# DogRog/no-time-to-train

Measured on NVIDIA B200. Metric: matching_stage_images_per_s, higher is better.
Workload: dtype f32

## Files before the change

no-time-to-train_b200/csrc/common.cuh:

```cuda
#pragma once

#include <cuda_runtime.h>
#include <stdint.h>

#include <atomic>

#include "../../include/nttt_b200.h"

namespace nttt {

constexpr int kWarp = 32;
constexpr unsigned kFull = 0xffffffffu;

int cuda_fail(cudaError_t e, const char* what);
#define NTTT_CUDA(expr)                                        \
  do {                                                         \
    cudaError_t _e = (expr);                                   \
    if (_e != cudaSuccess) return ::nttt::cuda_fail(_e, #expr); \
  } while (0)
cudaError_t set_dyn_smem_impl(const void* fn, int bytes);
template <typename F>
inline cudaError_t set_dyn_smem(F* fn, int bytes) { return set_dyn_smem_impl(reinterpret_cast<const void*>(fn), bytes); }
extern thread_local bool t_low_latency;
extern thread_local bool t_chain_break;
// ... 64 lines not shown
        __syncthreads();
        other = s_x[i ^ j];
        __syncthreads();
      } else {
        other = __shfl_xor_sync(kFull, key, j);
      }
      const bool take_min = ((i & j) == 0) == ((i & k) == 0);
      key = (take_min == (other < key)) ? other : key;
    }
  }
  return key;
}

__device__ __forceinline__ float4 ld_stream(const float4* p) {
  float4 r;
  asm volatile("ld.global.nc.L1::no_allocate.v4.f32 {%0,%1,%2,%3}, [%4];"
               : "=f"(r.x), "=f"(r.y), "=f"(r.z), "=f"(r.w)
               : "l"(p));
  return r;
}

struct AxisTable {
  int in_size = 0, out_size = 0, taps = 0;
  void* slab = nullptr;
  int32_t* xmin = nullptr;
  int32_t* xsize = nullptr;
  float* w = nullptr;
  int32_t* t_lo = nullptr;
  int32_t* t_len = nullptr;
  float* t_w = nullptr;
  float* t_cum = nullptr;
  int32_t* grp_of = nullptr;
  int32_t* grp_start = nullptr;
  float4* pk = nullptr;
};
constexpr int kGrpMax = 4;
constexpr int kMaxScatter = 24;

int aa_max_taps(int in_size, int out_size);

constexpr int kMaxChunks = 64;
struct ChunkTable {
  const float* base[kMaxChunks];
};

int build_axis_table(AxisTable& t, int in_size, int out_size, cudaStream_t s);
void free_axis_table(AxisTable& t);

}

struct nttt_ctx {
  int device = 0;
  int sm_count = 0;
  static constexpr int kMaxTables = 1024;
  static constexpr int kMaxRetired = 64;
  nttt::AxisTable tables[kMaxTables];
  unsigned long long last_use[kMaxTables] = {};
  nttt::AxisTable retired[kMaxRetired];
  int n_retired = 0;
  int max_tables = kMaxTables;
  unsigned long long epoch = 0;
  int n_tables = 0;
  int upsample_stage_floats = 36 * 1024 / 4;
  bool pool_order = true;
  int32_t* scratch = nullptr;
  size_t scratch_cap = 0;
  static constexpr int kMaxStages = 16;
// ... 20 lines not shown
```

no-time-to-train_b200/csrc/fullres.cu:

```cuda
#include "common.cuh"

namespace nttt {

constexpr int kUpThreads = 128;
constexpr int kUpMaxSplit = 8;
constexpr int kUpCols = 8;
constexpr int kUpSub = 32 / kUpCols;
constexpr int kUpGroupsPerCta = 32;

struct UpTables {
  const int32_t* xmin; const int32_t* xsize; const float* wx; int tx;
  const int32_t* ymin; const int32_t* ysize; const float* wy; int ty;
  const int32_t* x_tlo; const int32_t* x_tlen;
  const int32_t* y_tlo; const int32_t* y_tlen;
  const int32_t* y_grp_of; const int32_t* y_grp_start;
  const float4* pk_x; const float4* pk_y;
};

__device__ __forceinline__ float aa_dot(const float* __restrict__ src, int stride, const float* __restrict__ w, int n) {
  float acc = __fmul_rn(__ldg(src), __ldg(w));
  for (int j = 1; j < n; ++j) acc = __fmaf_rn(__ldg(src + (size_t)j * stride), __ldg(w + j), acc);
  return acc;
}

constexpr int kScratchInts = 8;
constexpr int kBig = 1 << 30;
constexpr int kTapsReg = 4;

struct alignas(16) UpMeta {
  const float* logits;
  int src;
  int safe;
  int r0, r1;
  int w0, w1;
  int lr0, lr1;
  int g0, g1;
};

__global__ void __launch_bounds__(256)
upsample_meta_kernel(const uint32_t* __restrict__ bits_lr, const int32_t* __restrict__ box_lr,
                     const int32_t* __restrict__ flags_lr, int ih, int iw, const int32_t* __restrict__ sel,
                     const int32_t* __restrict__ n_sel, int max_sel, UpTables t, UpMeta* __restrict__ meta,
                     int32_t* __restrict__ rect, int32_t* __restrict__ scratch, const float* __restrict__ logits,
                     const float* const* __restrict__ mask_ptr) {
  const int k = blockIdx.x * blockDim.x + threadIdx.x;
  if (k >= max_sel) return;
#pragma unroll
  for (int q = 0; q < kScratchInts; ++q) scratch[(size_t)k * kScratchInts + q] = 0;
  if (k >= min(*n_sel, max_sel)) return;
// ... 32 lines not shown
}
__device__ __forceinline__ void cp_async_wait_all() { asm volatile("cp.async.wait_all;" ::: "memory"); }

__global__ void __launch_bounds__(kUpThreads, 5)
upsample_pack_kernel(const uint32_t* __restrict__ bits_lr, const UpMeta* __restrict__ meta, int ih, int iw,
                     const int32_t* __restrict__ n_sel, int max_sel, int oh, int ow, UpTables t,
                     uint32_t* __restrict__ bits_full, int32_t* __restrict__ area_full, int32_t* __restrict__ box_full,
                     int32_t* __restrict__ scratch, int stage_floats) {
  extern __shared__ __align__(16) uint32_t s_lr[];
  __shared__ int s_red[5];
  const int k = blockIdx.y;
  if (k >= min(*n_sel, max_sel)) return;
  const UpMeta mt = meta[k];
  const int n_groups = mt.g1 - mt.g0;
  const int needed = up_ctas_needed(n_groups);
  if ((int)blockIdx.x >= needed) return;
  const int lr_wpr = iw >> 5;
  const int ow_words = (ow + 31) >> 5;
  const int lane = lane_id(), warp = warp_id();
  constexpr int kWarps = kUpThreads / 32;
  const int r0 = mt.r0, r1 = mt.r1, w0 = mt.w0, w1 = mt.w1;
  const int chunk0 = mt.g0 + blockIdx.x * kUpGroupsPerCta;
  const bool one_chunk = needed * kUpGroupsPerCta >= n_groups;

  int clr0 = mt.lr0, clr1 = mt.lr1;
  if (one_chunk && chunk0 < mt.g1) {
    const int gl = min(chunk0 + kUpGroupsPerCta, mt.g1);
    const int ya = max(t.y_grp_start[chunk0], r0), yb = min(t.y_grp_start[gl], r1);
    clr0 = t.ymin[ya];
    clr1 = t.ymin[yb - 1] + t.ysize[yb - 1];
  }
  const uint32_t* lr = bits_lr + ((size_t)mt.src * ih + clr0) * lr_wpr;
  const int n_lr = (clr1 - clr0) * lr_wpr;
  const bool fast_cfg = t.pk_x != nullptr && t.pk_y != nullptr;
  const float* src = mt.logits;
  float* tile = reinterpret_cast<float*>(s_lr + (((ih * lr_wpr + 1) + 3) & ~3));
  int tc0 = 0, tstride = 0;
  bool staged = false;
  if (fast_cfg && one_chunk && chunk0 < mt.g1 && stage_floats > 0 && w1 > w0) {
    const int xa = min(w0 << 5, ow - 1), xb = min((w1 << 5) - 1, ow - 1);
    tc0 = t.xmin[xa] & ~3;
    tstride = min((t.xmin[xb] + t.xsize[xb] + 3) & ~3, iw) - tc0;
    staged = tstride > 0 && (clr1 - clr0) * tstride <= stage_floats;
  }
  if (staged) {
    const int cpr = tstride >> 2;
    const int n_chunks = (clr1 - clr0) * cpr;
    const float* g0p = src + (size_t)clr0 * iw + tc0;
    for (int i = threadIdx.x; i < n_chunks; i += kUpThreads) {
      const int row = i / cpr, c4 = (i - row * cpr) << 2;
      cp_async16(tile + row * tstride + c4, g0p + (size_t)row * iw + c4);
    }
  }
  for (int i = threadIdx.x; i < n_lr; i += kUpThreads) s_lr[i] = lr[i];
  if (threadIdx.x < 5) s_red[threadIdx.x] = 0;
  const bool safe = mt.safe != 0;
  const float* tap_base = staged ? tile - clr0 * tstride : src;
  const int tap_stride = staged ? tstride : iw;
  const int tap_c0 = staged ? tc0 : 0;
  uint32_t* dst = bits_full + (size_t)k * oh * ow_words;
  cp_async_wait_all();
  __syncthreads();

  int area = 0, minx = kBig, maxx = -1, miny = kBig, maxy = -1;
  const int q = lane / kUpCols;
  for (int wbase = w0; wbase < w1; wbase += kUpCols) {
    const int wi = wbase + (lane & (kUpCols - 1));
    const bool active = wi < w1;
    const int x0 = min(wi << 5, ow - 1);
    const int x1 = min(x0 + 31, ow - 1);
    const uint32_t valid = (x1 - x0 == 31) ? 0xffffffffu : ((1u << (x1 - x0 + 1)) - 1u);
    const int c0 = t.xmin[x0];
    const int c1 = t.xmin[x1] + t.xsize[x1];
    const int cw0 = c0 >> 5;
    const bool two_words = ((c1 - 1) >> 5) <= cw0 + 1;
    uint32_t m0, m1 = 0;
    {
      const int lo = c0 - (cw0 << 5), hi = min(c1 - (cw0 << 5), 32);
      m0 = (hi - lo == 32) ? 0xffffffffu : (((1u << (hi - lo)) - 1u) << lo);
      const int hi1 = c1 - ((cw0 + 1) << 5);
      if (hi1 > 0) m1 = hi1 >= 32 ? 0xffffffffu : ((1u << hi1) - 1u);
    }
    uint32_t colbits = 0;
    for (int cb = chunk0; cb < mt.g1; cb += needed * kUpGroupsPerCta) {
      const int cend = min(cb + kUpGroupsPerCta, mt.g1);
      for (int g0 = cb + warp; g0 < cend; g0 += kWarps * kUpSub) {
        const int g = g0 + kWarps * q;
        const bool gvalid = g < cend;
        const int ya = gvalid ? max(t.y_grp_start[g], r0) : r0, yb = gvalid ? min(t.y_grp_start[g + 1], r1) : r0;
        const int nrows = yb - ya;
        int ry0, rys;
        if (fast_cfg) {
          const int pky = __float_as_int(__ldg(t.pk_y + (uint32_t)ya).x);
          ry0 = pky & 0xffff;
          rys = pky >> 16;
        } else {
          ry0 = t.ymin[ya];
          rys = t.ysize[ya];
        }
        const int rb = ry0 * tap_stride - tap_c0;
        const int lrb = (ry0 - clr0) * lr_wpr + cw0;
        uint32_t words[kGrpMax];
#pragma unroll
        for (int j = 0; j < kGrpMax; ++j) words[j] = 0;
        bool mixed = false;
        if (active && gvalid) {
          bool all0 = true, all1 = true;
          if (two_words) {
            uint32_t any = 0, miss = 0;
            if (rys <= 3) {
#pragma unroll
              for (int r = 0; r < 3; ++r) {
                if (r < rys) {
                  const uint32_t v0 = s_lr[(uint32_t)(lrb + r * lr_wpr)] & m0;
                  const uint32_t v1 = s_lr[(uint32_t)(lrb + r * lr_wpr + 1)] & m1;
                  any |= v0 | v1;
                  miss |= (v0 ^ m0) | (v1 ^ m1);
                }
              }
            } else {
              for (int r = 0; r < rys; ++r) {
                const uint32_t v0 = s_lr[lrb + r * lr_wpr] & m0;
                const uint32_t v1 = s_lr[lrb + r * lr_wpr + 1] & m1;
                any |= v0 | v1;
                miss |= (v0 ^ m0) | (v1 ^ m1);
              }
            }
            all0 = any == 0;
            all1 = miss == 0;
          } else {
            for (int r = 0; r < rys; ++r) {
              const uint32_t* row = s_lr + (lrb - cw0) + r * lr_wpr;
              for (int cw = cw0; cw <= (c1 - 1) >> 5; ++cw) {
                const int lo = max(c0 - (cw << 5), 0), hi = min(c1 - (cw << 5), 32);
                const uint32_t m = (hi - lo == 32) ? 0xffffffffu : (((1u << (hi - lo)) - 1u) << lo);
                const uint32_t v = row[cw] & m;
                all0 = all0 && (v == 0);
                all1 = all1 && (v == m);
              }
            }
          }
          if (all1 && safe && !all0) {
#pragma unroll
            for (int j = 0; j < kGrpMax; ++j) words[j] = valid;
          } else if (!all0) {
            mixed = true;
          }
        }
        uint32_t todo = __ballot_sync(kFull, mixed);
        while (todo) {
          const int src_lane = __ffs(todo) - 1;
          todo &= todo - 1;
          const int s_ya = __shfl_sync(kFull, ya, src_lane), s_nrows = __shfl_sync(kFull, nrows, src_lane);
          const int s_rb = __shfl_sync(kFull, rb, src_lane), s_rys = __shfl_sync(kFull, rys, src_lane);
          const int x = ((wbase + (src_lane & (kUpCols - 1))) << 5) + lane;
          if (fast_cfg) {
            const float4 xt = __ldg(t.pk_x + (uint32_t)x);
            const int pk = __float_as_int(xt.x);
            const int cx = pk & 0xffff, cs = pk >> 16;
            float T[3];
#pragma unroll
            for (int r = 0; r < 3; ++r) {
              float acc = 0.0f;
              if (r < s_rys) {
                const float* pl = tap_base + (s_rb + max(cx, tap_c0) + r * tap_stride);
                acc = __fmul_rn(*pl, xt.y);
                if (cs > 1) acc = __fmaf_rn(pl[1], xt.z, acc);
                if (cs > 2) acc = __fmaf_rn(pl[2], xt.w, acc);
              }
              T[r] = acc;
            }
#pragma unroll
            for (int j = 0; j < kGrpMax; ++j) {
              const float4 wv = __ldg(t.pk_y + (uint32_t)min(s_ya + j, s_ya + s_nrows - 1));
              float acc = __fmul_rn(T[0], wv.y);
              acc = __fmaf_rn(T[1], wv.z, acc);
              acc = __fmaf_rn(T[2], wv.w, acc);
              const uint32_t res = __ballot_sync(kFull, cs > 0 && acc > 0.0f);
              if (lane == src_lane) words[j] = res;
            }
            continue;
          }
          const bool inb = x < ow;
          const int cx = inb ? t.xmin[x] : 0, cs = inb ? t.xsize[x] : 1;
          const float* wx = t.wx + (size_t)(inb ? x : 0) * t.tx;
          const float* p = src + (s_rb + cx);
          if (s_rys <= kTapsReg) {
            float T[kTapsReg];
#pragma unroll
            for (int r = 0; r < kTapsReg; ++r) T[r] = (r < s_rys && inb) ? aa_dot(p + (size_t)r * iw, 1, wx, cs) : 0.0f;
#pragma unroll
            for (int j = 0; j < kGrpMax; ++j) {
              if (j < s_nrows) {
                const float* wy = t.wy + (size_t)(s_ya + j) * t.ty;
                float acc = __fmul_rn(T[0], __ldg(wy));
#pragma unroll
                for (int r = 1; r < kTapsReg; ++r)
                  if (r < s_rys) acc = __fmaf_rn(T[r], __ldg(wy + r), acc);
                const uint32_t res = __ballot_sync(kFull, inb && acc > 0.0f);
                if (lane == src_lane) words[j] = res;
              }
            }
          } else {
#pragma unroll
            for (int j = 0; j < kGrpMax; ++j) {
              if (j < s_nrows) {
                const float* wy = t.wy + (size_t)(s_ya + j) * t.ty;
                float acc = 0.0f;
                if (inb) {
                  acc = __fmul_rn(aa_dot(p, 1, wx, cs), __ldg(wy));
// ... 204 lines not shown
      const int tc0 = __ldg(t.xmin + xa) & ~3;
      const int tstride = min((__ldg(t.xmin + xb) + __ldg(t.xsize + xb) + 3) & ~3, iw) - tc0;
      Up2Item it;
      it.k = k0 + lo;
      it.g = gA | ((gB - gA) << 16);
      it.w = wA | ((wB - wA) << 16);
      it.y = ya | ((yb - ya) << 16);
      it.lr = l0 | ((l1 - l0) << 16);
      it.tc = tc0 | (tstride << 16);
      it.staged = (l1 - l0) * tstride <= tile_cap_floats ? 1 : 0;
      it.pad = 0;
      items[base + e] = it;
    }
    base += strip_items;
    __syncthreads();
  }
  if (blockIdx.x == 0 && tid == 0) { ctr[0] = base; ctr[1] = 0; }
}

__device__ __forceinline__ void cp_async16_ca(void* smem_dst, const void* gmem_src) {
  const uint32_t d = (uint32_t)__cvta_generic_to_shared(smem_dst);
  asm volatile("cp.async.ca.shared.global [%0], [%1], 16;" ::"r"(d), "l"(gmem_src) : "memory");
}
__device__ __forceinline__ void cp_async4(void* smem_dst, const void* gmem_src) {
  const uint32_t d = (uint32_t)__cvta_generic_to_shared(smem_dst);
  asm volatile("cp.async.ca.shared.global [%0], [%1], 4;" ::"r"(d), "l"(gmem_src) : "memory");
}
__device__ __forceinline__ float lds_f32(uint32_t saddr) {
  float v;
  asm volatile("ld.shared.f32 %0, [%1];" : "=f"(v) : "r"(saddr));
  return v;
}

template <bool kStaged>
__device__ __forceinline__ float up2_row(const float* __restrict__ gsrc, uint32_t saddr, int idx, const float4& xt, int cs) {
  float a0, a1 = 0.0f, a2 = 0.0f;
  if (kStaged) {
    const uint32_t p = saddr + ((uint32_t)idx << 2);
    a0 = lds_f32(p);
    if (cs > 1) a1 = lds_f32(p + 4);
    if (cs > 2) a2 = lds_f32(p + 8);
  } else {
    const float* p = gsrc + idx;
    a0 = __ldg(p);
    if (cs > 1) a1 = __ldg(p + 1);
    if (cs > 2) a2 = __ldg(p + 2);
  }
  float acc = __fmul_rn(a0, xt.y);
  acc = __fmaf_rn(a1, xt.z, acc);
  acc = __fmaf_rn(a2, xt.w, acc);
  return acc;
}

struct alignas(16) Up2Group { int row, nrows, trow, rys; };

template <bool kStaged>
__device__ __forceinline__ void up2_evaluate(int warp, int lane, int n_list, const uint16_t* __restrict__ s_list,
                                             const Up2Group* __restrict__ s_grp, const float4* __restrict__ s_pkx,
                                             const float4* __restrict__ s_pky, uint32_t* __restrict__ s_out,
                                             const float* __restrict__ gsrc, uint32_t tile_saddr, int tap_stride,
                                             int tap_c0) {
  constexpr int kWarps = kUp2Threads / 32;
  for (int e = warp; e < n_list; e += kWarps) {
    const int ent = s_list[e];
    const int u = ent >> 5, gl = ent & 31;
    const Up2Group g = s_grp[gl];
    const float4 xt = s_pkx[(u << 5) + lane];
    const int pk = __float_as_int(xt.x);
    const int cx = pk & 0xffff, cs = pk >> 16;
    const int idx = g.trow + max(cx - tap_c0, 0);
    const float T0 = up2_row<kStaged>(gsrc, tile_saddr, idx, xt, cs);
    float T1 = 0.0f, T2 = 0.0f;
    if (g.rys > 1) T1 = up2_row<kStaged>(gsrc, tile_saddr, idx + tap_stride, xt, cs);
    if (g.rys > 2) T2 = up2_row<kStaged>(gsrc, tile_saddr, idx + 2 * tap_stride, xt, cs);
    const float4* wy = s_pky + g.row;
    uint32_t mine = 0;
#pragma unroll
    for (int j = 0; j < kGrpMax; ++j) {
      const float4 wv = wy[j];
      float acc = __fmul_rn(T0, wv.y);
      acc = __fmaf_rn(T1, wv.z, acc);
      acc = __fmaf_rn(T2, wv.w, acc);
      const uint32_t res = __ballot_sync(kFull, cs > 0 && acc > 0.0f);
      if (lane == j) mine = res;
    }
    if (lane < g.nrows) {
      const int row = g.row + lane;
      s_out[u * kUp2OutStride + row + (row >> 5)] = mine;
    }
  }
}

__global__ void __launch_bounds__(kUp2Threads, kUp2CtasPerSm)
upsample_pack2_kernel(const uint32_t* __restrict__ bits_lr, const UpMeta* __restrict__ meta, int ih, int iw, int oh,
                      int ow, UpTables t, uint32_t* __restrict__ bits_full, uint32_t* __restrict__ bits_t,
                      int32_t* __restrict__ area_full, int32_t* __restrict__ box_full, int32_t* __restrict__ scratch,
                      const Up2Item* __restrict__ items, int32_t* __restrict__ ctr, int32_t* __restrict__ zero2) {
  chain_wait();
  if (zero2 && blockIdx.x == 0 && threadIdx.x == 0) { zero2[0] = 0; zero2[1] = 0; }
  extern __shared__ __align__(16) unsigned char s_raw[];
  float4* s_pkx = reinterpret_cast<float4*>(s_raw);
  float4* s_pky = s_pkx + kUp2Cols * 32;
  Up2Group* s_grp = reinterpret_cast<Up2Group*>(s_pky + kUp2Rows + kGrpMax);
  uint32_t* s_out = reinterpret_cast<uint32_t*>(s_grp + kUp2Groups);
  int* s_gstart = reinterpret_cast<int*>(s_out + kUp2Cols * kUp2OutStride);
  uint16_t* s_list = reinterpret_cast<uint16_t*>(s_gstart + kUp2Groups + 4);
  const int lr_wpr = iw >> 5;
  uint32_t* s_lr = reinterpret_cast<uint32_t*>(s_list + kUp2Cols * kUp2Groups);
  float* tile = reinterpret_cast<float*>(s_lr + ((ih * lr_wpr + 4 + 3) & ~3));
  __shared__ int s_item;
  __shared__ int s_red[5];
  __shared__ uint32_t s_mix[kUp2Cols];
  const int tid = threadIdx.x, lane = tid & 31, warp = tid >> 5;
  constexpr int kWarps = kUp2Threads / 32;
  const int ow_words = (ow + 31) >> 5;
  const int total = ctr[0];
  const uint32_t tile_saddr = (uint32_t)__cvta_generic_to_shared(tile);
  for (;;) {
    __syncthreads();
    if (tid == 0) s_item = atomicAdd(&ctr[1], 1);
    if (tid < 5) s_red[tid] = 0;
    __syncthreads();
    const int item = s_item;
    if (item >= total) break;
    const Up2Item it = items[item];
    const int k = it.k;
    const UpMeta mt = meta[k];
    const int gA = it.g & 0xffff, ng = it.g >> 16;
    const int wA = it.w & 0xffff, nw = it.w >> 16;
    const int ya0 = it.y & 0xffff, n_rows = it.y >> 16;
    const int clr0 = it.lr & 0xffff, tr = it.lr >> 16;
    const int tc0 = it.tc & 0xffff, tstride = it.tc >> 16;
    const bool staged = it.staged != 0;
    const float* src = mt.logits;
    if (staged) {
      const int cpr = tstride >> 2;
      const float* gp = src + (size_t)(clr0 + warp) * iw + tc0 + (lane << 2);
      uint32_t sp = tile_saddr + (uint32_t)((warp * tstride + (lane << 2)) << 2);
      const uint32_t sp_step = (uint32_t)(kWarps * tstride) << 2;
      const size_t gp_step = (size_t)kWarps * iw;
      for (int row = warp; row < tr; row += kWarps, gp += gp_step, sp += sp_step)
        for (int c = lane; c < cpr; c += 32)
          asm volatile("cp.async.cg.shared.global [%0], [%1], 16;" ::"r"(sp + ((uint32_t)(c - lane) << 4)), "l"(gp + ((c - lane) << 2)) : "memory");
    }
    {
      const uint32_t* lr = bits_lr + ((size_t)mt.src * ih + clr0) * lr_wpr;
      const int n_lr = tr * lr_wpr;
      if ((lr_wpr & 3) == 0 && (reinterpret_cast<uintptr_t>(lr) & 15) == 0) {
        for (int i = tid; i < (n_lr >> 2); i += kUp2Threads) cp_async16_ca(s_lr + 4 * i, lr + 4 * i);
      } else {
        for (int i = tid; i < n_lr; i += kUp2Threads) cp_async4(s_lr + i, lr + i);
      }
      for (int i = tid; i < n_rows; i += kUp2Threads) cp_async16_ca(s_pky + i, t.pk_y + ya0 + i);
      const float4* px = t.pk_x + (wA << 5);
      for (int i = tid; i < (nw << 5); i += kUp2Threads) cp_async16_ca(s_pkx + i, px + i);
      if (tid <= ng) s_gstart[tid] = min(max(t.y_grp_start[gA + tid], mt.r0), mt.r1);
    }
    cp_async_wait_all();
    __syncthreads();
    const int tap_stride = staged ? tstride : iw;
    const int tap_c0 = staged ? tc0 : 0;
    const bool safe = mt.safe != 0;
    int my_ya = 0, my_nrows = 0, my_ry0 = 0, my_rys = 0;
    if (lane < ng) {
      my_ya = s_gstart[lane];
      my_nrows = s_gstart[lane + 1] - my_ya;
      if (my_nrows > 0) {
        const int pky = __float_as_int(s_pky[my_ya - ya0].x);
        my_ry0 = pky & 0xffff;
        my_rys = pky >> 16;
      }
      if (warp == 0) {
        Up2Group g;
        g.row = my_ya - ya0;
        g.nrows = my_nrows;
        g.trow = (staged ? my_ry0 - clr0 : my_ry0) * tap_stride;
        g.rys = my_rys;
        s_grp[lane] = g;
      }
    }
    for (int u = warp; u < nw; u += kWarps) {
      const int wi = wA + u;
      const int x0 = min(wi << 5, ow - 1);
      const int x1 = min(x0 + 31, ow - 1);
      const uint32_t valid = (x1 - x0 == 31) ? 0xffffffffu : ((1u << (x1 - x0 + 1)) - 1u);
      const int p0 = __float_as_int(s_pkx[x0 - (wA << 5)].x), p1 = __float_as_int(s_pkx[x1 - (wA << 5)].x);
      const int c0 = p0 & 0xffff;
      const int c1 = (p1 & 0xffff) + (p1 >> 16);
      const int cw0 = c0 >> 5;
      const bool two_words = ((c1 - 1) >> 5) <= cw0 + 1;
      uint32_t m0, m1 = 0;
      {
        const int lo = c0 - (cw0 << 5), hi = min(c1 - (cw0 << 5), 32);
        m0 = (hi - lo == 32) ? 0xffffffffu : (((1u << (hi - lo)) - 1u) << lo);
        const int hi1 = c1 - ((cw0 + 1) << 5);
        if (hi1 > 0) m1 = hi1 >= 32 ? 0xffffffffu : ((1u << hi1) - 1u);
      }
      int cls = 0;
      if (my_nrows > 0) {
        const int lrb = (my_ry0 - clr0) * lr_wpr + cw0;
        bool all0 = true, all1 = true;
        if (two_words) {
          uint32_t any = 0, miss = 0;
          for (int r = 0; r < my_rys; ++r) {
            const uint32_t v0 = s_lr[lrb + r * lr_wpr] & m0;
            const uint32_t v1 = s_lr[lrb + r * lr_wpr + 1] & m1;
            any |= v0 | v1;
            miss |= (v0 ^ m0) | (v1 ^ m1);
          }
          all0 = any == 0;
          all1 = miss == 0;
        } else {
          for (int r = 0; r < my_rys; ++r) {
            const uint32_t* row = s_lr + (lrb - cw0) + r * lr_wpr;
            for (int cw = cw0; cw <= (c1 - 1) >> 5; ++cw) {
              const int lo = max(c0 - (cw << 5), 0), hi = min(c1 - (cw << 5), 32);
              const uint32_t m = (hi - lo == 32) ? 0xffffffffu : (((1u << (hi - lo)) - 1u) << lo);
              const uint32_t v = row[cw] & m;
              all0 = all0 && (v == 0);
              all1 = all1 && (v == m);
            }
          }
        }
        cls = all0 ? 0 : ((all1 && safe) ? 1 : 2);
        if (cls != 2) {
          const uint32_t word = cls == 1 ? valid : 0u;
          const int row = my_ya - ya0;
          for (int j = 0; j < my_nrows; ++j) s_out[u * kUp2OutStride + (row + j) + ((row + j) >> 5)] = word;
        }
      }
      const uint32_t mixed = __ballot_sync(kFull, cls == 2);
      if (lane == 0) s_mix[u] = mixed;
    }
    __syncthreads();
    int n_list = 0;
    {
      int off = 0;
      for (int u = 0; u < nw; ++u) {
        const uint32_t mixed = s_mix[u];
        if ((u & (kWarps - 1)) == warp && ((mixed >> lane) & 1u))
          s_list[off + __popc(mixed & ((1u << lane) - 1u))] = (uint16_t)((u << 5) | lane);
        off += __popc(mixed);
      }
      n_list = off;
    }
    __syncthreads();
    if (staged)
      up2_evaluate<true>(warp, lane, n_list, s_list, s_grp, s_pkx, s_pky, s_out, src, tile_saddr, tap_stride, tap_c0);
    else
      up2_evaluate<false>(warp, lane, n_list, s_list, s_grp, s_pkx, s_pky, s_out, src, tile_saddr, tap_stride, tap_c0);
    __syncthreads();
    if (bits_t) {
      uint32_t* dt = bits_t + (size_t)k * oh * ow_words;
      for (int c = warp; c < nw; c += kWarps)
        for (int row = lane; row < n_rows; row += 32)
          dt[(uint32_t)((wA + c) * oh + ya0 + row)] = s_out[c * kUp2OutStride + row + (row >> 5)];
    }
    {
      uint32_t* dst = bits_full ? bits_full + (size_t)k * oh * ow_words : nullptr;
      const int c = tid & (kUp2Cols - 1);
      int area = 0, miny = kBig, maxy = -1;
      uint32_t colbits = 0;
      if (c < nw) {
        for (int row = tid >> 3; row < n_rows; row += kUp2Threads / kUp2Cols) {
          const uint32_t w = s_out[c * kUp2OutStride + row + (row >> 5)];
          if (dst) dst[(uint32_t)((ya0 + row) * ow_words + wA + c)] = w;
          area += __popc(w);
          colbits |= w;
          if (w) { miny = min(miny, ya0 + row); maxy = max(maxy, ya0 + row); }
        }
      }
      int minx = kBig, maxx = -1;
      if (colbits) {
        minx = ((wA + c) << 5) + __ffs(colbits) - 1;
        maxx = ((wA + c) << 5) + 31 - __clz(colbits);
      }
      area = warp_sum(area);
      minx = warp_min(minx); miny = warp_min(miny); maxx = warp_max(maxx); maxy = warp_max(maxy);
      if (lane == 0) {
        atomicAdd(&s_red[0], area);
        atomicMax(&s_red[1], maxx + 1);
        atomicMax(&s_red[2], maxy + 1);
        atomicMax(&s_red[3], kBig - minx);
        atomicMax(&s_red[4], kBig - miny);
      }
    }
    __syncthreads();
    if (tid == 0) {
      int32_t* sc = scratch + (size_t)k * kScratchInts;
      atomicAdd(&sc[0], s_red[0]);
      atomicMax(&sc[1], s_red[1]);
      atomicMax(&sc[2], s_red[2]);
      atomicMax(&sc[3], s_red[3]);
      atomicMax(&sc[4], s_red[4]);
      __threadfence();
      const int prev = atomicAdd(&sc[5], 1);
      if (prev == sc[6] - 1) {
        __threadfence();
        const int a = atomicAdd(&sc[0], 0);
        const int mx1 = atomicMax(&sc[1], 0), my1 = atomicMax(&sc[2], 0);
        const int bx = atomicMax(&sc[3], 0), by = atomicMax(&sc[4], 0);
        area_full[k] = a;
        int4 o = make_int4(0, 0, 0, 0);
        if (a > 0) o = make_int4(kBig - bx, kBig - by, mx1 - 1, my1 - 1);
        reinterpret_cast<int4*>(box_full)[k] = o;
      }
    }
  }
}

static size_t up2_fixed_smem(int ih, int iw) {
  const size_t lr_words = (((size_t)ih * (iw / 32) + 4) + 3) & ~(size_t)3;
  return sizeof(float4) * (kUp2Cols * 32 + kUp2Rows + kGrpMax + kUp2Groups) +
         4 * ((size_t)kUp2Cols * kUp2OutStride + kUp2Groups + 4 + lr_words) + 2 * (size_t)kUp2Cols * kUp2Groups;
}
static size_t up2_max_items(int max_sel, int oh, int ow) {
  return (size_t)max_sel * ((oh + kUp2Groups - 1) / kUp2Groups) * ((((ow + 31) / 32) + kUp2Cols - 1) / kUp2Cols);
}

int launch_upsample_pack(const AxisTable& tx, const AxisTable& ty, const float* logits, const uint32_t* bits_lr,
                         const int32_t* box_lr, const int32_t* flags_lr, int ih, int iw, const int32_t* sel,
                         const int32_t* n_sel, int max_sel, int oh, int ow, uint32_t* bits_full, int32_t* rect,
                         int32_t* area_full, int32_t* box_full, int32_t* scratch, const float* const* mask_ptr,
                         cudaStream_t s, int stage_floats, int sm_count, uint32_t* bits_t, bool* wrote_t, bool t_only,
                         bool low_latency, int32_t* zero2) {
  if (wrote_t) *wrote_t = false;
  if (max_sel <= 0) return NTTT_OK;
  if (iw % 32 != 0) return NTTT_EUNSUPPORTED;
  UpTables t{tx.xmin, tx.xsize, tx.w, tx.taps, ty.xmin, ty.xsize, ty.w, ty.taps, tx.t_lo, tx.t_len, ty.t_lo, ty.t_len,
             ty.grp_of, ty.grp_start, tx.pk, ty.pk};
  UpMeta* meta = reinterpret_cast<UpMeta*>(scratch + (size_t)kScratchInts * max_sel);
  if (tx.pk && ty.pk && oh < 65536 && ow < 65536 && ih * (iw / 32) <= 16384) {
    int32_t* ctr = reinterpret_cast<int32_t*>(meta + max_sel);
    Up2Item* items = reinterpret_cast<Up2Item*>(ctr + 4);
    const double sy = (double)ih / oh, sx = (double)iw / ow;
    long need = (long)((kUp2Rows * sy + 6)) * (long)(((kUp2Cols * 32) * sx + 12));
    int tile_floats = (int)(need < stage_floats ? need : stage_floats);
    if (tile_floats < 0) tile_floats = 0;
    tile_floats = (tile_floats + 3) & ~3;
    const size_t smem = up2_fixed_smem(ih, iw) + (size_t)tile_floats * 4;
    if (smem > 200 * 1024) return NTTT_EUNSUPPORTED;
    launch_chain(upsample_plan_kernel, 8, kPlanThreads, 0, s, bits_lr, box_lr, flags_lr, ih, iw, sel, n_sel, max_sel, t, meta, rect,
                                                    scratch, logits, mask_ptr, items, ctr, area_full, box_full, oh, ow,
                                                    tile_floats);
    NTTT_LAUNCH_CHECK();
    if (smem > 48 * 1024)
      NTTT_CUDA(set_dyn_smem(upsample_pack2_kernel, (int)smem));
    const int grid = (sm_count > 0 ? sm_count : 148) * (low_latency ? kUp2CtasPerSm : 1);
    launch_chain(upsample_pack2_kernel, grid, kUp2Threads, smem, s, bits_lr, meta, ih, iw, oh, ow, t,
                                                          (bits_t && t_only) ? nullptr : bits_full, bits_t, area_full,
                                                          box_full, scratch, items, ctr, zero2);
    NTTT_LAUNCH_CHECK();
    if (wrote_t) *wrote_t = bits_t != nullptr;
    return NTTT_OK;
  }
  const size_t bits_bytes = ((((size_t)ih * (iw / 32) + 1) + 3) & ~(size_t)3) * 4;
  if (bits_bytes > 160 * 1024) return NTTT_EUNSUPPORTED;
  size_t stage_bytes = (size_t)(stage_floats > 0 ? stage_floats : 0) * 4;
  if (bits_bytes + stage_bytes > 200 * 1024) stage_bytes = 0;
  const size_t smem = bits_bytes + stage_bytes;
  if (smem > 48 * 1024)
    NTTT_CUDA(set_dyn_smem(upsample_pack_kernel, (int)smem));
  upsample_meta_kernel<<<ceil_div(max_sel, 256), 256, 0, s>>>(bits_lr, box_lr, flags_lr, ih, iw, sel, n_sel, max_sel, t,
                                                              meta, rect, scratch, logits, mask_ptr);
  NTTT_LAUNCH_CHECK();
// ... 133 lines not shown
```

no-time-to-train_b200/csrc/lowres.cu:

```cuda
#include <cuda_bf16.h>
#include <stdlib.h>

#include "common.cuh"

namespace nttt {

constexpr int kPackThreads = 256;
constexpr int kPackBlock = kPackThreads + 32;
constexpr int kPackStages = 4;
constexpr int kPackStageF4 = 4 * kPackThreads;
constexpr int kPackStageBytes = kPackStageF4 * 16;

__device__ __forceinline__ uint32_t pk_smem_u32(const void* p) { return (uint32_t)__cvta_generic_to_shared(p); }
__device__ __forceinline__ void pk_mbar_init(uint64_t* bar, uint32_t count) {
  asm volatile("mbarrier.init.shared::cta.b64 [%0], %1;" ::"r"(pk_smem_u32(bar)), "r"(count));
}
__device__ __forceinline__ void pk_mbar_expect_tx(uint32_t bar_addr, uint32_t bytes) {
  asm volatile("mbarrier.arrive.expect_tx.shared::cta.b64 _, [%0], %1;" ::"r"(bar_addr), "r"(bytes) : "memory");
}
__device__ __forceinline__ void pk_mbar_arrive(uint32_t bar_addr) {
  asm volatile("mbarrier.arrive.shared::cta.b64 _, [%0];" ::"r"(bar_addr) : "memory");
}
__device__ __forceinline__ void pk_mbar_wait(uint32_t bar_addr, uint32_t parity) {
  for (uint32_t spin = 0; spin < (1u << 20); ++spin) {
    uint32_t done;
    asm volatile(
        "{\n\t.reg .pred p;\n\t"
        "mbarrier.try_wait.parity.shared::cta.b64 p, [%1], %2, %3;\n\t"
        "selp.u32 %0, 1, 0, p;\n\t}"
        : "=r"(done)
        : "r"(bar_addr), "r"(parity), "r"(4000u)
        : "memory");
    if (done) return;
  }
// ... 583 lines not shown
    }
  }
  const int len = lo < 0 ? 0 : hi - lo + 1;
  t_lo[e] = max(lo, 0);
  t_len[e] = len;
  for (int t = 0; t < kMaxScatter; ++t) {
    const int x = lo + t;
    float v = 0.0f;
    if (lo >= 0 && x <= hi && e >= xmin[x] && e < xmin[x] + xsize[x]) v = w[(size_t)x * taps + (e - xmin[x])];
    t_w[(size_t)e * kMaxScatter + t] = v;
  }
  float c = 0.0f;
  t_cum[(size_t)e * (kMaxScatter + 1)] = 0.0f;
  for (int t = 0; t < kMaxScatter; ++t) {
    c += t_w[(size_t)e * kMaxScatter + t];
    t_cum[(size_t)e * (kMaxScatter + 1) + t + 1] = c;
  }
}

__global__ void aa_group_kernel(int out_size, const int32_t* xmin, const int32_t* xsize, int32_t* grp_of,
                                int32_t* grp_start) {
  if (blockIdx.x != 0 || threadIdx.x != 0) return;
  int g = -1, run = 0;
  for (int i = 0; i < out_size; ++i) {
    const bool same = i > 0 && xmin[i] == xmin[i - 1] && xsize[i] == xsize[i - 1] && run < kGrpMax;
    if (!same) { ++g; grp_start[g] = i; run = 0; }
    grp_of[i] = g;
    ++run;
  }
  for (int k = g + 1; k <= out_size; ++k) grp_start[k] = out_size;
}

__global__ void aa_pack_kernel(int out_size, int out_pad, int taps, const int32_t* xmin, const int32_t* xsize,
                               const float* w, float4* pk) {
  const int i = blockIdx.x * blockDim.x + threadIdx.x;
  if (i >= out_pad) return;
  float4 e = make_float4(0.f, 0.f, 0.f, 0.f);
  if (i < out_size) {
    const int cs = xsize[i];
    const float* wi = w + (size_t)i * taps;
    e.x = __int_as_float(xmin[i] | (cs << 16));
    e.y = cs > 0 ? wi[0] : 0.0f;
    e.z = cs > 1 ? wi[1] : 0.0f;
    e.w = cs > 2 ? wi[2] : 0.0f;
  }
  pk[i] = e;
}

int build_axis_table(AxisTable& t, int in_size, int out_size, cudaStream_t s) {
  t.in_size = in_size;
  t.out_size = out_size;
  t.taps = aa_max_taps(in_size, out_size);
  const bool packed = t.taps <= 3 && in_size < 65536;
  const int out_pad = (out_size + 31) / 32 * 32;
  size_t off = 0;
  auto take = [&](size_t bytes) { const size_t o = off; off = align_up(off + bytes, 256); return o; };
  const size_t o_xmin = take(sizeof(int32_t) * out_size), o_xsize = take(sizeof(int32_t) * out_size);
  const size_t o_w = take(sizeof(float) * (size_t)out_size * t.taps);
  const size_t o_tlo = take(sizeof(int32_t) * in_size), o_tlen = take(sizeof(int32_t) * in_size);
  const size_t o_tw = take(sizeof(float) * (size_t)in_size * kMaxScatter);
  const size_t o_tcum = take(sizeof(float) * (size_t)in_size * (kMaxScatter + 1));
  const size_t o_gof = take(sizeof(int32_t) * out_size), o_gst = take(sizeof(int32_t) * ((size_t)out_size + 1));
  const size_t o_pk = packed ? take(sizeof(float4) * (size_t)out_pad) : 0;
  char* slab = nullptr;
  NTTT_CUDA(cudaMalloc(&slab, off));
  t.slab = slab;
  t.xmin = reinterpret_cast<int32_t*>(slab + o_xmin);
  t.xsize = reinterpret_cast<int32_t*>(slab + o_xsize);
  t.w = reinterpret_cast<float*>(slab + o_w);
  t.t_lo = reinterpret_cast<int32_t*>(slab + o_tlo);
  t.t_len = reinterpret_cast<int32_t*>(slab + o_tlen);
  t.t_w = reinterpret_cast<float*>(slab + o_tw);
  t.t_cum = reinterpret_cast<float*>(slab + o_tcum);
  t.grp_of = reinterpret_cast<int32_t*>(slab + o_gof);
  t.grp_start = reinterpret_cast<int32_t*>(slab + o_gst);
  t.pk = packed ? reinterpret_cast<float4*>(slab + o_pk) : nullptr;
  aa_table_kernel<<<ceil_div(out_size, 128), 128, 0, s>>>(in_size, out_size, t.taps, t.xmin, t.xsize, t.w);
  NTTT_LAUNCH_CHECK();
  aa_transpose_kernel<<<ceil_div(in_size, 128), 128, 0, s>>>(in_size, out_size, t.taps, t.xmin, t.xsize, t.w, t.t_lo,
                                                            t.t_len, t.t_w, t.t_cum);
  NTTT_LAUNCH_CHECK();
  aa_group_kernel<<<1, 32, 0, s>>>(out_size, t.xmin, t.xsize, t.grp_of, t.grp_start);
  NTTT_LAUNCH_CHECK();
  if (packed) {
    aa_pack_kernel<<<ceil_div(out_pad, 128), 128, 0, s>>>(out_size, out_pad, t.taps, t.xmin, t.xsize, t.w, t.pk);
    NTTT_LAUNCH_CHECK();
  }
  return NTTT_OK;
}

void free_axis_table(AxisTable& t) {
  if (t.slab) cudaFree(t.slab);
  t = AxisTable{};
}

constexpr int kProjThreads = 256;

struct ProjTables {
  const int32_t* x_lo; const int32_t* x_len; const float* x_cum;
  const int32_t* y_lo; const int32_t* y_len; const float* y_w;
};

__device__ __forceinline__ void split_bf16_pair(float x, __nv_bfloat16& hi, __nv_bfloat16& lo) {
  hi = __float2bfloat16_rn(x);
  lo = __float2bfloat16_rn(x - __bfloat162float(hi));
}

constexpr int kCum = kMaxScatter + 1;
constexpr int kProjRows = 64;

template <typename F>
__device__ __forceinline__ void warp_range(int n, F flag, int& lo, int& hi) {
  const int lane = lane_id();
  const uint32_t b0 = __ballot_sync(kFull, lane < n && flag(lane));
  const uint32_t b1 = __ballot_sync(kFull, lane + 32 < n && flag(lane + 32));
  lo = b0 ? __ffs(b0) - 1 : (b1 ? 32 + __ffs(b1) - 1 : 1);
  hi = b1 ? 63 - __clz(b1) : (b0 ? 31 - __clz(b0) : 0);
}
// ... 227 lines not shown
```

Measured before the change: 12080.

## Split packed resize tables into span and 2-tap weights; defer scratch publish

Replaces the float4 packed axis table with a separate uint32 span array and a float2 weight array. The packed path is now enabled only when every output's support spans at most two input taps, so the upsample evaluation drops the third tap and does fewer loads and FMAs. The persistent upsample loop now prefetches the next work item early and defers the global atomic publish of the previous item so it overlaps the next item's loads. The bits_t and bits_full store passes are also merged with the area and box reduction. In exchange, the fast path covers fewer scale configurations, and the host-side float check must match the device tap computation exactly.

```diff
diff --git a/no-time-to-train_b200/csrc/common.cuh b/no-time-to-train_b200/csrc/common.cuh
--- a/no-time-to-train_b200/csrc/common.cuh
+++ b/no-time-to-train_b200/csrc/common.cuh
@@ -120,7 +120,8 @@
   float* t_cum = nullptr;
   int32_t* grp_of = nullptr;
   int32_t* grp_start = nullptr;
-  float4* pk = nullptr;
+  uint32_t* pk_span = nullptr;
+  float2* pk_w = nullptr;
 };
 constexpr int kGrpMax = 4;
 constexpr int kMaxScatter = 24;
diff --git a/no-time-to-train_b200/csrc/fullres.cu b/no-time-to-train_b200/csrc/fullres.cu
--- a/no-time-to-train_b200/csrc/fullres.cu
+++ b/no-time-to-train_b200/csrc/fullres.cu
@@ -14,7 +14,7 @@
   const int32_t* x_tlo; const int32_t* x_tlen;
   const int32_t* y_tlo; const int32_t* y_tlen;
   const int32_t* y_grp_of; const int32_t* y_grp_start;
-  const float4* pk_x; const float4* pk_y;
+  const uint32_t* pkx_span; const float2* pkx_w; const uint32_t* pky_span; const float2* pky_w;
 };
 
 __device__ __forceinline__ float aa_dot(const float* __restrict__ src, int stride, const float* __restrict__ w, int n) {
@@ -113,7 +113,7 @@
   }
   const uint32_t* lr = bits_lr + ((size_t)mt.src * ih + clr0) * lr_wpr;
   const int n_lr = (clr1 - clr0) * lr_wpr;
-  const bool fast_cfg = t.pk_x != nullptr && t.pk_y != nullptr;
+  const bool fast_cfg = t.pkx_span != nullptr && t.pky_span != nullptr;
   const float* src = mt.logits;
   float* tile = reinterpret_cast<float*>(s_lr + (((ih * lr_wpr + 1) + 3) & ~3));
   int tc0 = 0, tstride = 0;
@@ -172,7 +172,7 @@
         const int nrows = yb - ya;
         int ry0, rys;
         if (fast_cfg) {
-          const int pky = __float_as_int(__ldg(t.pk_y + (uint32_t)ya).x);
+          const int pky = (int)__ldg(t.pky_span + (uint32_t)ya);
           ry0 = pky & 0xffff;
           rys = pky >> 16;
         } else {
@@ -236,27 +236,25 @@
           const int s_rb = __shfl_sync(kFull, rb, src_lane), s_rys = __shfl_sync(kFull, rys, src_lane);
           const int x = ((wbase + (src_lane & (kUpCols - 1))) << 5) + lane;
           if (fast_cfg) {
-            const float4 xt = __ldg(t.pk_x + (uint32_t)x);
-            const int pk = __float_as_int(xt.x);
+            const float2 xt = __ldg(t.pkx_w + (uint32_t)x);
+            const int pk = (int)__ldg(t.pkx_span + (uint32_t)x);
             const int cx = pk & 0xffff, cs = pk >> 16;
-            float T[3];
-#pragma unroll
-            for (int r = 0; r < 3; ++r) {
+            float T[2];
+#pragma unroll
+            for (int r = 0; r < 2; ++r) {
               float acc = 0.0f;
               if (r < s_rys) {
                 const float* pl = tap_base + (s_rb + max(cx, tap_c0) + r * tap_stride);
-                acc = __fmul_rn(*pl, xt.y);
-                if (cs > 1) acc = __fmaf_rn(pl[1], xt.z, acc);
-                if (cs > 2) acc = __fmaf_rn(pl[2], xt.w, acc);
+                acc = __fmul_rn(*pl, xt.x);
+                if (cs > 1) acc = __fmaf_rn(pl[1], xt.y, acc);
               }
               T[r] = acc;
             }
 #pragma unroll
             for (int j = 0; j < kGrpMax; ++j) {
-              const float4 wv = __ldg(t.pk_y + (uint32_t)min(s_ya + j, s_ya + s_nrows - 1));
-              float acc = __fmul_rn(T[0], wv.y);
-              acc = __fmaf_rn(T[1], wv.z, acc);
-              acc = __fmaf_rn(T[2], wv.w, acc);
+              const float2 wv = __ldg(t.pky_w + (uint32_t)min(s_ya + j, s_ya + s_nrows - 1));
+              float acc = __fmul_rn(T[0], wv.x);
+              acc = __fmaf_rn(T[1], wv.y, acc);
               const uint32_t res = __ballot_sync(kFull, cs > 0 && acc > 0.0f);
               if (lane == src_lane) words[j] = res;
             }
@@ -527,55 +525,49 @@
   return v;
 }
 
+
 template <bool kStaged>
-__device__ __forceinline__ float up2_row(const float* __restrict__ gsrc, uint32_t saddr, int idx, const float4& xt, int cs) {
-  float a0, a1 = 0.0f, a2 = 0.0f;
+__device__ __forceinline__ float up2_row(const float* __restrict__ gsrc, uint32_t saddr, int idx, const float2& wx, int cs) {
+  float a0, a1 = 0.0f;
   if (kStaged) {
     const uint32_t p = saddr + ((uint32_t)idx << 2);
     a0 = lds_f32(p);
     if (cs > 1) a1 = lds_f32(p + 4);
-    if (cs > 2) a2 = lds_f32(p + 8);
   } else {
     const float* p = gsrc + idx;
     a0 = __ldg(p);
     if (cs > 1) a1 = __ldg(p + 1);
-    if (cs > 2) a2 = __ldg(p + 2);
-  }
-  float acc = __fmul_rn(a0, xt.y);
-  acc = __fmaf_rn(a1, xt.z, acc);
-  acc = __fmaf_rn(a2, xt.w, acc);
-  return acc;
+  }
+  return __fmaf_rn(a1, wx.y, __fmul_rn(a0, wx.x));
 }
 
 struct alignas(16) Up2Group { int row, nrows, trow, rys; };
 
 template <bool kStaged>
 __device__ __forceinline__ void up2_evaluate(int warp, int lane, int n_list, const uint16_t* __restrict__ s_list,
-                                             const Up2Group* __restrict__ s_grp, const float4* __restrict__ s_pkx,
-                                             const float4* __restrict__ s_pky, uint32_t* __restrict__ s_out,
-                                             const float* __restrict__ gsrc, uint32_t tile_saddr, int tap_stride,
-                                             int tap_c0) {
+                                             const Up2Group* __restrict__ s_grp, const uint32_t* __restrict__ s_xspan,
+                                             const float2* __restrict__ s_xw, const float2* __restrict__ s_yw,
+                                             uint32_t* __restrict__ s_out, const float* __restrict__ gsrc,
+                                             uint32_t tile_saddr, int tap_stride, int tap_c0) {
   constexpr int kWarps = kUp2Threads / 32;
   for (int e = warp; e < n_list; e += kWarps) {
     const int ent = s_list[e];
     const int u = ent >> 5, gl = ent & 31;
     const Up2Group g = s_grp[gl];
-    const float4 xt = s_pkx[(u << 5) + lane];
-    const int pk = __float_as_int(xt.x);
+    const int px = (u << 5) + lane;
+    const int pk = (int)s_xspan[px];
+    const float2 wx = s_xw[px];
     const int cx = pk & 0xffff, cs = pk >> 16;
     const int idx = g.trow + max(cx - tap_c0, 0);
-    const float T0 = up2_row<kStaged>(gsrc, tile_saddr, idx, xt, cs);
-    float T1 = 0.0f, T2 = 0.0f;
-    if (g.rys > 1) T1 = up2_row<kStaged>(gsrc, tile_saddr, idx + tap_stride, xt, cs);
-    if (g.rys > 2) T2 = up2_row<kStaged>(gsrc, tile_saddr, idx + 2 * tap_stride, xt, cs);
-    const float4* wy = s_pky + g.row;
+    const float T0 = up2_row<kStaged>(gsrc, tile_saddr, idx, wx, cs);
+    const float T1r = up2_row<kStaged>(gsrc, tile_saddr, idx + (g.rys > 1 ? tap_stride : 0), wx, cs);
+    const float T1 = g.rys > 1 ? T1r : 0.0f;
+    const float2* wy = s_yw + g.row;
     uint32_t mine = 0;
 #pragma unroll
     for (int j = 0; j < kGrpMax; ++j) {
-      const float4 wv = wy[j];
-      float acc = __fmul_rn(T0, wv.y);
-      acc = __fmaf_rn(T1, wv.z, acc);
-      acc = __fmaf_rn(T2, wv.w, acc);
+      const float2 wv = wy[j];
+      const float acc = __fmaf_rn(T1, wv.y, __fmul_rn(T0, wv.x));
       const uint32_t res = __ballot_sync(kFull, cs > 0 && acc > 0.0f);
       if (lane == j) mine = res;
     }
@@ -583,6 +575,28 @@
       const int row = g.row + lane;
       s_out[u * kUp2OutStride + row + (row >> 5)] = mine;
     }
+  }
+}
+
+__device__ __forceinline__ void up2_publish(int k, const int (&red)[5], int32_t* __restrict__ scratch,
+                                            int32_t* __restrict__ area_full, int32_t* __restrict__ box_full) {
+  int32_t* sc = scratch + (size_t)k * kScratchInts;
+  atomicAdd(&sc[0], red[0]);
+  atomicMax(&sc[1], red[1]);
+  atomicMax(&sc[2], red[2]);
+  atomicMax(&sc[3], red[3]);
+  atomicMax(&sc[4], red[4]);
+  __threadfence();
+  const int prev = atomicAdd(&sc[5], 1);
+  if (prev == sc[6] - 1) {
+    __threadfence();
+    const int a = atomicAdd(&sc[0], 0);
+    const int mx1 = atomicMax(&sc[1], 0), my1 = atomicMax(&sc[2], 0);
+    const int bx = atomicMax(&sc[3], 0), by = atomicMax(&sc[4], 0);
+    area_full[k] = a;
+    int4 o = make_int4(0, 0, 0, 0);
+    if (a > 0) o = make_int4(kBig - bx, kBig - by, mx1 - 1, my1 - 1);
+    reinterpret_cast<int4*>(box_full)[k] = o;
   }
 }
 
@@ -594,9 +608,11 @@
   chain_wait();
   if (zero2 && blockIdx.x == 0 && threadIdx.x == 0) { zero2[0] = 0; zero2[1] = 0; }
   extern __shared__ __align__(16) unsigned char s_raw[];
-  float4* s_pkx = reinterpret_cast<float4*>(s_raw);
-  float4* s_pky = s_pkx + kUp2Cols * 32;
-  Up2Group* s_grp = reinterpret_cast<Up2Group*>(s_pky + kUp2Rows + kGrpMax);
+  float2* s_xw = reinterpret_cast<float2*>(s_raw);
+  float2* s_yw = s_xw + kUp2Cols * 32;
+  uint32_t* s_xspan = reinterpret_cast<uint32_t*>(s_yw + kUp2Rows + 8);
+  uint32_t* s_yspan = s_xspan + kUp2Cols * 32;
+  Up2Group* s_grp = reinterpret_cast<Up2Group*>(s_yspan + kUp2Rows + 4);
   uint32_t* s_out = reinterpret_cast<uint32_t*>(s_grp + kUp2Groups);
   int* s_gstart = reinterpret_cast<int*>(s_out + kUp2Cols * kUp2OutStride);
   uint16_t* s_list = reinterpret_cast<uint16_t*>(s_gstart + kUp2Groups + 4);
@@ -611,13 +627,14 @@
   const int ow_words = (ow + 31) >> 5;
   const int total = ctr[0];
   const uint32_t tile_saddr = (uint32_t)__cvta_generic_to_shared(tile);
+  int next = 0, pend_k = -1, pend[5];
+  if (tid == 0) s_item = atomicAdd(&ctr[1], 1);
   for (;;) {
-    __syncthreads();
-    if (tid == 0) s_item = atomicAdd(&ctr[1], 1);
-    if (tid < 5) s_red[tid] = 0;
     __syncthreads();
     const int item = s_item;
     if (item >= total) break;
+    if (tid == 0) next = atomicAdd(&ctr[1], 1);
+    if (tid < 5) s_red[tid] = 0;
     const Up2Item it = items[item];
     const int k = it.k;
     const UpMeta mt = meta[k];
@@ -646,11 +663,14 @@
       } else {
         for (int i = tid; i < n_lr; i += kUp2Threads) cp_async4(s_lr + i, lr + i);
       }
-      for (int i = tid; i < n_rows; i += kUp2Threads) cp_async16_ca(s_pky + i, t.pk_y + ya0 + i);
-      const float4* px = t.pk_x + (wA << 5);
-      for (int i = tid; i < (nw << 5); i += kUp2Threads) cp_async16_ca(s_pkx + i, px + i);
+      const int yb = ya0 & ~3, ny = n_rows + (ya0 & 3);
+      for (int i = tid; i < ((ny + 3) >> 2); i += kUp2Threads) cp_async16_ca(s_yspan + 4 * i, t.pky_span + yb + 4 * i);
+      for (int i = tid; i < ((ny + 1) >> 1); i += kUp2Threads) cp_async16_ca(s_yw + 2 * i, t.pky_w + yb + 2 * i);
+      for (int i = tid; i < (nw << 3); i += kUp2Threads) cp_async16_ca(s_xspan + 4 * i, t.pkx_span + (wA << 5) + 4 * i);
+      for (int i = tid; i < (nw << 4); i += kUp2Threads) cp_async16_ca(s_xw + 2 * i, t.pkx_w + (wA << 5) + 2 * i);
       if (tid <= ng) s_gstart[tid] = min(max(t.y_grp_start[gA + tid], mt.r0), mt.r1);
     }
+    if (tid == 0 && pend_k >= 0) up2_publish(pend_k, pend, scratch, area_full, box_full);
     cp_async_wait_all();
     __syncthreads();
     const int tap_stride = staged ? tstride : iw;
@@ -661,7 +681,7 @@
       my_ya = s_gstart[lane];
       my_nrows = s_gstart[lane + 1] - my_ya;
       if (my_nrows > 0) {
-        const int pky = __float_as_int(s_pky[my_ya - ya0].x);
+        const int pky = (int)s_yspan[my_ya - (ya0 & ~3)];
         my_ry0 = pky & 0xffff;
         my_rys = pky >> 16;
       }
@@ -679,7 +699,7 @@
       const int x0 = min(wi << 5, ow - 1);
       const int x1 = min(x0 + 31, ow - 1);
       const uint32_t valid = (x1 - x0 == 31) ? 0xffffffffu : ((1u << (x1 - x0 + 1)) - 1u);
-      const int p0 = __float_as_int(s_pkx[x0 - (wA << 5)].x), p1 = __float_as_int(s_pkx[x1 - (wA << 5)].x);
+      const int p0 = (int)s_xspan[x0 - (wA << 5)], p1 = (int)s_xspan[x1 - (wA << 5)];
       const int c0 = p0 & 0xffff;
       const int c1 = (p1 & 0xffff) + (p1 >> 16);
       const int cw0 = c0 >> 5;
@@ -741,34 +761,50 @@
     }
     __syncthreads();
     if (staged)
-      up2_evaluate<true>(warp, lane, n_list, s_list, s_grp, s_pkx, s_pky, s_out, src, tile_saddr, tap_stride, tap_c0);
+      up2_evaluate<true>(warp, lane, n_list, s_list, s_grp, s_xspan, s_xw, s_yw + (ya0 & 3), s_out, src, tile_saddr,
+                         tap_stride, tap_c0);
     else
-      up2_evaluate<false>(warp, lane, n_list, s_list, s_grp, s_pkx, s_pky, s_out, src, tile_saddr, tap_stride, tap_c0);
+      up2_evaluate<false>(warp, lane, n_list, s_list, s_grp, s_xspan, s_xw, s_yw + (ya0 & 3), s_out, src, tile_saddr,
+                          tap_stride, tap_c0);
     __syncthreads();
-    if (bits_t) {
-      uint32_t* dt = bits_t + (size_t)k * oh * ow_words;
-      for (int c = warp; c < nw; c += kWarps)
-        for (int row = lane; row < n_rows; row += 32)
-          dt[(uint32_t)((wA + c) * oh + ya0 + row)] = s_out[c * kUp2OutStride + row + (row >> 5)];
-    }
     {
-      uint32_t* dst = bits_full ? bits_full + (size_t)k * oh * ow_words : nullptr;
-      const int c = tid & (kUp2Cols - 1);
-      int area = 0, miny = kBig, maxy = -1;
-      uint32_t colbits = 0;
-      if (c < nw) {
-        for (int row = tid >> 3; row < n_rows; row += kUp2Threads / kUp2Cols) {
-          const uint32_t w = s_out[c * kUp2OutStride + row + (row >> 5)];
-          if (dst) dst[(uint32_t)((ya0 + row) * ow_words + wA + c)] = w;
-          area += __popc(w);
-          colbits |= w;
-          if (w) { miny = min(miny, ya0 + row); maxy = max(maxy, ya0 + row); }
-        }
-      }
-      int minx = kBig, maxx = -1;
-      if (colbits) {
-        minx = ((wA + c) << 5) + __ffs(colbits) - 1;
-        maxx = ((wA + c) << 5) + 31 - __clz(colbits);
+      int area = 0, minx = kBig, maxx = -1, miny = kBig, maxy = -1;
+      if (bits_t) {
+        uint32_t* dt = bits_t + (size_t)k * oh * ow_words;
+        for (int c = warp; c < nw; c += kWarps) {
+          uint32_t colbits = 0;
+          for (int row = lane; row < n_rows; row += 32) {
+            const uint32_t w = s_out[c * kUp2OutStride + row + (row >> 5)];
+            dt[(uint32_t)((wA + c) * oh + ya0 + row)] = w;
+            area += __popc(w);
+            colbits |= w;
+            if (w) { miny = min(miny, ya0 + row); maxy = max(maxy, ya0 + row); }
+          }
+          if (colbits) {
+            minx = min(minx, ((wA + c) << 5) + __ffs(colbits) - 1);
+            maxx = max(maxx, ((wA + c) << 5) + 31 - __clz(colbits));
+          }
+        }
+      }
+      if (bits_full) {
+        uint32_t* dst = bits_full + (size_t)k * oh * ow_words;
+        const int c = tid & (kUp2Cols - 1);
+        uint32_t colbits = 0;
+        if (c < nw) {
+          for (int row = tid >> 3; row < n_rows; row += kUp2Threads / kUp2Cols) {
+            const uint32_t w = s_out[c * kUp2OutStride + row + (row >> 5)];
+            dst[(uint32_t)((ya0 + row) * ow_words + wA + c)] = w;
+            if (!bits_t) {
+              area += __popc(w);
+              colbits |= w;
+              if (w) { miny = min(miny, ya0 + row); maxy = max(maxy, ya0 + row); }
+            }
+          }
+        }
+        if (colbits) {
+          minx = ((wA + c) << 5) + __ffs(colbits) - 1;
+          maxx = ((wA + c) << 5) + 31 - __clz(colbits);
+        }
       }
       area = warp_sum(area);
       minx = warp_min(minx); miny = warp_min(miny); maxx = warp_max(maxx); maxy = warp_max(maxy);
@@ -782,31 +818,19 @@
     }
     __syncthreads();
     if (tid == 0) {
-      int32_t* sc = scratch + (size_t)k * kScratchInts;
-      atomicAdd(&sc[0], s_red[0]);
-      atomicMax(&sc[1], s_red[1]);
-      atomicMax(&sc[2], s_red[2]);
-      atomicMax(&sc[3], s_red[3]);
-      atomicMax(&sc[4], s_red[4]);
-      __threadfence();
-      const int prev = atomicAdd(&sc[5], 1);
-      if (prev == sc[6] - 1) {
-        __threadfence();
-        const int a = atomicAdd(&sc[0], 0);
-        const int mx1 = atomicMax(&sc[1], 0), my1 = atomicMax(&sc[2], 0);
-        const int bx = atomicMax(&sc[3], 0), by = atomicMax(&sc[4], 0);
-        area_full[k] = a;
-        int4 o = make_int4(0, 0, 0, 0);
-        if (a > 0) o = make_int4(kBig - bx, kBig - by, mx1 - 1, my1 - 1);
-        reinterpret_cast<int4*>(box_full)[k] = o;
-      }
-    }
-  }
+      pend_k = k;
+#pragma unroll
+      for (int q = 0; q < 5; ++q) pend[q] = s_red[q];
+      s_item = next;
+    }
+  }
+  if (tid == 0 && pend_k >= 0) up2_publish(pend_k, pend, scratch, area_full, box_full);
 }
 
 static size_t up2_fixed_smem(int ih, int iw) {
   const size_t lr_words = (((size_t)ih * (iw / 32) + 4) + 3) & ~(size_t)3;
-  return sizeof(float4) * (kUp2Cols * 32 + kUp2Rows + kGrpMax + kUp2Groups) +
+  return (sizeof(float2) + sizeof(uint32_t)) * (kUp2Cols * 32 + kUp2Rows + 4) + sizeof(float2) * 4 +
+         sizeof(Up2Group) * kUp2Groups +
          4 * ((size_t)kUp2Cols * kUp2OutStride + kUp2Groups + 4 + lr_words) + 2 * (size_t)kUp2Cols * kUp2Groups;
 }
 static size_t up2_max_items(int max_sel, int oh, int ow) {
@@ -823,9 +847,9 @@
   if (max_sel <= 0) return NTTT_OK;
   if (iw % 32 != 0) return NTTT_EUNSUPPORTED;
   UpTables t{tx.xmin, tx.xsize, tx.w, tx.taps, ty.xmin, ty.xsize, ty.w, ty.taps, tx.t_lo, tx.t_len, ty.t_lo, ty.t_len,
-             ty.grp_of, ty.grp_start, tx.pk, ty.pk};
+             ty.grp_of, ty.grp_start, tx.pk_span, tx.pk_w, ty.pk_span, ty.pk_w};
   UpMeta* meta = reinterpret_cast<UpMeta*>(scratch + (size_t)kScratchInts * max_sel);
-  if (tx.pk && ty.pk && oh < 65536 && ow < 65536 && ih * (iw / 32) <= 16384) {
+  if (tx.pk_span && ty.pk_span && oh < 65536 && ow < 65536 && ih * (iw / 32) <= 16384) {
     int32_t* ctr = reinterpret_cast<int32_t*>(meta + max_sel);
     Up2Item* items = reinterpret_cast<Up2Item*>(ctr + 4);
     const double sy = (double)ih / oh, sx = (double)iw / ow;
diff --git a/no-time-to-train_b200/csrc/lowres.cu b/no-time-to-train_b200/csrc/lowres.cu
--- a/no-time-to-train_b200/csrc/lowres.cu
+++ b/no-time-to-train_b200/csrc/lowres.cu
@@ -1,5 +1,7 @@
 #include <cuda_bf16.h>
 #include <stdlib.h>
+
+#include <algorithm>
 
 #include "common.cuh"
 
@@ -649,26 +651,39 @@
 }
 
 __global__ void aa_pack_kernel(int out_size, int out_pad, int taps, const int32_t* xmin, const int32_t* xsize,
-                               const float* w, float4* pk) {
+                               const float* w, uint32_t* pk_span, float2* pk_w) {
   const int i = blockIdx.x * blockDim.x + threadIdx.x;
   if (i >= out_pad) return;
-  float4 e = make_float4(0.f, 0.f, 0.f, 0.f);
+  uint32_t span = 0;
+  float2 e = make_float2(0.f, 0.f);
   if (i < out_size) {
     const int cs = xsize[i];
     const float* wi = w + (size_t)i * taps;
-    e.x = __int_as_float(xmin[i] | (cs << 16));
-    e.y = cs > 0 ? wi[0] : 0.0f;
-    e.z = cs > 1 ? wi[1] : 0.0f;
-    e.w = cs > 2 ? wi[2] : 0.0f;
-  }
-  pk[i] = e;
+    span = (uint32_t)xmin[i] | ((uint32_t)cs << 16);
+    e.x = cs > 0 ? wi[0] : 0.0f;
+    e.y = cs > 1 ? wi[1] : 0.0f;
+  }
+  pk_span[i] = span;
+  pk_w[i] = e;
+}
+
+static bool aa_spans_within_two(int in_size, int out_size) {
+  if (in_size > out_size) return false;
+  const float scale = (float)in_size / (float)out_size;
+  for (int i = 0; i < out_size; ++i) {
+    volatile float center = scale * ((float)i + 0.5f);
+    volatile float a = center - 1.0f, b = center + 1.0f;
+    const int lo = std::max((int)(a + 0.5f), 0), hi = std::min((int)(b + 0.5f), in_size);
+    if (hi - lo > 2) return false;
+  }
+  return true;
 }
 
 int build_axis_table(AxisTable& t, int in_size, int out_size, cudaStream_t s) {
   t.in_size = in_size;
   t.out_size = out_size;
   t.taps = aa_max_taps(in_size, out_size);
-  const bool packed = t.taps <= 3 && in_size < 65536;
+  const bool packed = in_size < 65536 && aa_spans_within_two(in_size, out_size);
   const int out_pad = (out_size + 31) / 32 * 32;
   size_t off = 0;
   auto take = [&](size_t bytes) { const size_t o = off; off = align_up(off + bytes, 256); return o; };
@@ -678,7 +693,8 @@
   const size_t o_tw = take(sizeof(float) * (size_t)in_size * kMaxScatter);
   const size_t o_tcum = take(sizeof(float) * (size_t)in_size * (kMaxScatter + 1));
   const size_t o_gof = take(sizeof(int32_t) * out_size), o_gst = take(sizeof(int32_t) * ((size_t)out_size + 1));
-  const size_t o_pk = packed ? take(sizeof(float4) * (size_t)out_pad) : 0;
+  const size_t o_pks = packed ? take(sizeof(uint32_t) * (size_t)out_pad) : 0;
+  const size_t o_pkw = packed ? take(sizeof(float2) * (size_t)out_pad) : 0;
   char* slab = nullptr;
   NTTT_CUDA(cudaMalloc(&slab, off));
   t.slab = slab;
@@ -691,7 +707,8 @@
   t.t_cum = reinterpret_cast<float*>(slab + o_tcum);
   t.grp_of = reinterpret_cast<int32_t*>(slab + o_gof);
   t.grp_start = reinterpret_cast<int32_t*>(slab + o_gst);
-  t.pk = packed ? reinterpret_cast<float4*>(slab + o_pk) : nullptr;
+  t.pk_span = packed ? reinterpret_cast<uint32_t*>(slab + o_pks) : nullptr;
+  t.pk_w = packed ? reinterpret_cast<float2*>(slab + o_pkw) : nullptr;
   aa_table_kernel<<<ceil_div(out_size, 128), 128, 0, s>>>(in_size, out_size, t.taps, t.xmin, t.xsize, t.w);
   NTTT_LAUNCH_CHECK();
   aa_transpose_kernel<<<ceil_div(in_size, 128), 128, 0, s>>>(in_size, out_size, t.taps, t.xmin, t.xsize, t.w, t.t_lo,
@@ -700,7 +717,8 @@
   aa_group_kernel<<<1, 32, 0, s>>>(out_size, t.xmin, t.xsize, t.grp_of, t.grp_start);
   NTTT_LAUNCH_CHECK();
   if (packed) {
-    aa_pack_kernel<<<ceil_div(out_pad, 128), 128, 0, s>>>(out_size, out_pad, t.taps, t.xmin, t.xsize, t.w, t.pk);
+    aa_pack_kernel<<<ceil_div(out_pad, 128), 128, 0, s>>>(out_size, out_pad, t.taps, t.xmin, t.xsize, t.w, t.pk_span,
+                                                             t.pk_w);
     NTTT_LAUNCH_CHECK();
   }
   return NTTT_OK;
```

After: 12460, median of 6. 1.03x the previous value.
